# cyrillefavreau/Sol-R

Hardware: AMD Instinct MI355X
Metric: Mrays/s @1920x1080, 3-bounce Cornell (higher is better)
Workload: dtype f32; 1 GPU; cornell 1920x1080, 3 bounces + shadow rays, 75 boxes / 29 primitives, one GPU, whole frame; rays_per_frame=6518779, closest_hit_walks_rank0=3506171, lane_nodes=206382796, lane_prim_tests=37557299, wave_nodes=3396811, wave_prim_tests=626627, wave_walks=106204, cost_ordered_launch_rank0=True, frames_in_flight=3, setup_frames_before_warmup=48, frames_delivered=9105, order_free_nodes=46, short_ray_lists=1, gather=none (one GPU), strips=equal rows, parallelism=tile1

## Files before the change

### sol-r_amd/csrc/build_bounds.h

```cpp
#ifndef SOLR_BUILD_BOUNDS_H
#define SOLR_BUILD_BOUNDS_H

#include <hip/hip_vector_types.h>

#include <cmath>
#include <cstring>

#include "../../include/solr_types.h"

#if defined(__HIPCC__)
#define SOLR_BUILD_BOUNDS_FN __host__ __device__ inline
#else
#define SOLR_BUILD_BOUNDS_FN inline
#endif

namespace solreng
{
#define SOLR_DOMINANT_SHARE 0.25

struct BuildBounds
{
    const float4 *prims = nullptr;
    float margin = 0.f;
    double dominantShare = SOLR_DOMINANT_SHARE;
};

enum BuildBoundsPlainKind
{
    BB_KIND_SHIFT = 24,
    BB_KIND_PLANE_XY = 2,
    BB_KIND_PLANE_YZ = 3,
    BB_KIND_PLANE_XZ = 4
};

SOLR_BUILD_BOUNDS_FN int centreBin(float c, float origin, float scale, int bins)
{
    const float at = (c - origin) * scale;
    const float last = (float)(bins - 1);
    return (int)(at > 0.f ? (at < last ? at : last) : 0.f);
}

SOLR_BUILD_BOUNDS_FN bool leafBuildBounds(const float4 &row0, const float4 &row1, const float4 *prims, int start, int count, float margin,
                                          float lo[3], float hi[3], bool byKind = false)
{
    lo[0] = row0.x, lo[1] = row0.y, lo[2] = row0.z;
    hi[0] = row1.x, hi[1] = row1.y, hi[2] = row0.w;
    if (prims == nullptr || count <= 0 || start < 0)
        return false;
    float lx = INFINITY, ly = INFINITY, lz = INFINITY, hx = -INFINITY, hy = -INFINITY, hz = -INFINITY;
    for (int k = 0; k < count; ++k)
    {
        const float4 p = prims[8 * (size_t)(start + k)], s = prims[8 * (size_t)(start + k) + 1];
        int word;
        memcpy(&word, &p.w, 4);
        const int type = word & 0xff, kind = (word >> BB_KIND_SHIFT) & 15;
        const int across = byKind ? (kind == BB_KIND_PLANE_YZ ? 0 : kind == BB_KIND_PLANE_XZ ? 1 : kind == BB_KIND_PLANE_XY ? 2 : -1)
                                  : (type == ptYZPlane ? 0 : type == ptXZPlane ? 1 : type == ptXYPlane ? 2 : -1);
        if (across < 0)
            return false;
        const float ex = across == 0 ? margin : fabsf(s.x) + margin;
        const float ey = across == 1 ? margin : fabsf(s.y) + margin;
        const float ez = across == 2 ? margin : fabsf(s.z) + margin;
        lx = fminf(lx, p.x - ex), hx = fmaxf(hx, p.x + ex);
        ly = fminf(ly, p.y - ey), hy = fmaxf(hy, p.y + ey);
        lz = fminf(lz, p.z - ez), hz = fmaxf(hz, p.z + ez);
    }
    if (!(lx <= hx && ly <= hy && lz <= hz && fabsf(lx) < 3.0e38f && fabsf(hx) < 3.0e38f && fabsf(ly) < 3.0e38f && fabsf(hy) < 3.0e38f &&
          fabsf(lz) < 3.0e38f && fabsf(hz) < 3.0e38f))
        return false;
    const float nlx = fmaxf(lo[0], lx), nly = fmaxf(lo[1], ly), nlz = fmaxf(lo[2], lz);
    const float nhx = fminf(hi[0], hx), nhy = fminf(hi[1], hy), nhz = fminf(hi[2], hz);
    if (!(nlx <= nhx && nly <= nhy && nlz <= nhz))
        return false;
    lo[0] = nlx, lo[1] = nly, lo[2] = nlz;
    hi[0] = nhx, hi[1] = nhy, hi[2] = nhz;
    return true;
}
}

#endif
```

### sol-r_amd/csrc/engine.h

```cpp
#ifndef SOLR_ENGINE_H
#define SOLR_ENGINE_H

#include <hip/hip_runtime.h>

#include <atomic>
#include <chrono>
#include <cstdio>
#include <cstdlib>
#include <cstring>
#include <string>
#include <vector>

#include "../../include/solr_hip.h"
#include "renderer.h"
#include "lists_device.h"
#include "list_builders.h"

namespace solreng
{
struct HostProfile
{
    const bool on = getenv("SOLR_HIP_HOST_PROFILE") != nullptr;
    struct Entry
    {
// ... 114 lines not shown
    static int ticketOf(long serial, int slot) { return (int)((serial % TICKET_PERIOD) * IMAGE_RING + slot); }
    long imageSerial = 0;
    long slotSerial[IMAGE_RING] = {};
    long shareSeq = 0;
    long slotShareSeq[IMAGE_RING] = {};
    long lastWaitedSeq = 0;
    long sharePublished[IMAGE_RING] = {};
    struct SharedRing *sharedRing = nullptr;
    size_t sharedBytes = 0;
    std::string sharedName;
    int shareRank = 0, shareWorld = 0;
    bool slotOfStrips[IMAGE_RING] = {};
    long lastHandedOut = 0;
    bool copyOnRenderStream = false;
    void release();
};
extern ImageRing gImageRing;
struct CopyLane
{
    hipStream_t stream = nullptr;
    hipEvent_t frameRendered = nullptr;
    hipEvent_t imageDone[ImageRing::IMAGE_RING] = {};
    void release();
};
struct ImageStreaming
{
    int next = 0;
    bool ids = false;
    bool valid = false;
    const void *bitmap = nullptr;
    unsigned serial = 0;
    long key[3] = {0, 0, 0};
    DeviceBuffer counters;
    StreamPlan plan = {};
    int bands = 0;
    unsigned *hostWords = nullptr;
    hipEvent_t rendered = nullptr;
    long delivered = 0;
    int support = -1;
    void release();
};
const int SORT_PERIOD = 64;

struct TileSchedule
{
    int mode = 1;
    DeviceBuffer cost, costSnapshot;
    DeviceBuffer order[2];
    int orderBuffer = 0;
    hipEvent_t orderEvent = nullptr;
    bool orderWait[MAX_FLIGHTS] = {};
    unsigned *hostStats = nullptr;
    unsigned *hostStatsDev = nullptr;
    long key[6] = {0, 0, 0, 0, 0, 0};
    int frames = 0;
    bool reorder = false;
    bool orderValid = false;
    BandCuts orderCuts = {};
    void reset()
    {
        frames = 0;
        reorder = false;
        orderValid = false;
    }
    void release();
};

enum Variant
{
    VARIANT_AUTOMATIC = 0,
    VARIANT_EXACT_LIST = 3,
    VARIANT_ALL_FEATURES = 4,
    VARIANT_NO_GROUPING = 5,
    VARIANT_NO_ORDER_FREE = 6,
    VARIANT_STACK_IN_LDS = 7,
    VARIANT_REFERENCE_LEAVES = 8,
    VARIANT_AO_FIXED_STRIDE = 9,
    VARIANT_NAN_DEEP_STACK = 10,
    VARIANT_UNSORTED_LISTS = 12,
    VARIANT_NO_BAND_WORDS = 13,
    VARIANT_ZERO_STREAM_COUNTERS = 14,
    VARIANT_NO_LAMP_CUTOFF = 15,
    VARIANT_ALL_TRIPS = 16,
    VARIANT_UPLOADED_BUILD_BOXES = 17
};

struct NodeList
{
    int copies, lists;
    explicit NodeList(int copies_ = 1, int lists_ = 1) : copies(copies_), lists(lists_) {}
    std::vector<float4> rows;
    std::vector<int> start, origin;
    int nb = 0;
    unsigned offRows = 0, offLeaf = 0;
    unsigned offStart = 0;
    int ordered = 0;
    bool tight = false;
    std::vector<int> refitLevels;

    void reset() { *this = NodeList(copies, lists); }
    unsigned nodes() const { return (unsigned)lists * (unsigned)nb; }
    unsigned rowsOf(int list) const { return solrdev::listRows(offRows, (unsigned)nb, (unsigned)list); }
    unsigned offThin() const { return solrdev::listThin(offRows, nodes()); }
    unsigned offSorted() const { return solrdev::listSorted(offRows, nodes()); }
    unsigned layRows(unsigned row)
    {
        offRows = row;
        return row + (unsigned)copies * solrdev::listCopyRows(nodes());
    }
    unsigned layStart(unsigned row)
    {
        offStart = row * 4;
        return row + (nodes() + 3u) / 4u;
    }
    unsigned layLeaf(unsigned row)
    {
        row = (row + 3u) & ~3u;
        offLeaf = row;
        return row + 4u * nodes() + 4u;
    }
};


struct Arena
{
    DeviceBuffer geometry;
    unsigned offPrims = 0, offLights = 0;
    unsigned rowsFixed = 0;
    bool geometryDirty = true;
    bool deviceAhead = false;
    void layOutAgain() { geometryDirty = true; }
};
struct OrderFreeState
{
    int freeCountdown = 0;
    bool freeHostValid = true;
    bool freeDirty = false;
    SolrDeviceLists freeStage;
    bool freeStale = false;
    bool sortedFree = false;
    void dropStage(bool originToo)
    {
        if (freeStage.rows)
            (void)hipFree(freeStage.rows);
        if (freeStage.start)
            (void)hipFree(freeStage.start);
        freeStage.rows = nullptr;
        freeStage.start = nullptr;
        if (originToo && freeStage.origin)
        {
            (void)hipFree(freeStage.origin);
            freeStage.origin = nullptr;
        }
    }
};
struct Rotation
{
    DeviceBuffer movable, refitPlan;
    DeviceBuffer enclosesFlag;
    int nbMovable = -1;
    bool refitReady = false;
    bool refitPlanPending = false;
    bool exactStale = false;
    float exactStaleViewDistance = 0.f;
    int nbDeviceRotations = 0;
    int nbDeviceTranslations = 0;
    int nbDeviceLampMoves = 0;
// ... 163 lines not shown
        if (slot < SOLR_MORPH_TRACK_MAX_KEYS)
            ++morph.nbTrackKeys;
    }
    void morphLampNoted(int slotA, int slotB, bool moves)
    {
        if (morph.lampChecked != retags)
            morph.lampAnswers.clear();
        morph.lampChecked = retags;
        morph.lampAnswers.push_back({slotA, slotB, moves});
    }
    void morphServed(bool walkHolds, bool landed, bool track)
    {
        walkEncloses = walkHolds;
        if (landed)
        {
            arena.deviceAhead = true;
            ++(track ? morph.nbDeviceTrackMorphs : morph.nbDeviceMorphs);
        }
    }
    void release()
    {
        lists.dropStage(true);
        for (DeviceBuffer *b : {&arena.geometry, &lamps, &rotation.movable, &rotation.refitPlan, &rotation.enclosesFlag, &rotation.edits,
                                &morph.lampFlag})
            solreng::release(*b);
        for (MorphKey &key : morph.keys)
            solreng::release(key.planes);
        *this = Scene();
    }
};
struct Lights
{
    std::vector<float4> hostLights;
    int nbLights = 0;
};
struct TextureUse
{
    int material;
    long texels;
    long offsets[7];
};
struct Materials
{
    DeviceBuffer table;
    unsigned offMatCold = 0;
    int nbMaterials = 0;
    std::vector<int> materialTags;
    std::vector<float> materialAverage;
    std::vector<TextureUse> textureUses;
    void release()
    {
        solreng::release(table);
        *this = Materials();
    }
};
struct Textures
{
    DeviceBuffer atlas;
    size_t atlasBytes = 0;
    bool textureTablesChecked = false;
    void release()
    {
        solreng::release(atlas);
        *this = Textures();
    }
};
struct Randoms
{
    DeviceBuffer values;
    long nbRandoms = 0;
    float randomsReach = 0.f;
    void release()
    {
        solreng::release(values);
        *this = Randoms();
    }
};
struct SceneFacts
{
    bool primsContained = false;
    bool opaqueShadows = false;
    bool plainPlanes = false;
    float sceneExtent = 1.f;
    int sceneFeatures = F_ALL & ~F_FULL;
};
struct KernelTimer
{
    unsigned timingTick = 0;
    std::vector<std::pair<hipEvent_t, hipEvent_t>> events;
    double timedMs = 0.0;
    int timedLaunches = 0;
    std::vector<float> kernelSamples, intervalSamples;
};
struct WalkRecording
{
    DeviceBuffer walkRecords, walkVisits;
    bool recordNext = false;
    bool recorded = false;
    unsigned recordGrid = 0;
    size_t recordLds = 0;
    int recordVariant = -1;
    bool recordDeep = false;
    SceneArgs recordScene = {};
    void release()
    {
        solreng::release(walkRecords);
        solreng::release(walkVisits);
        *this = WalkRecording();
    }
};

struct Engine
{
    bool initialized = false;
    int device = 0;
    int errorCode = 0;
    std::string errorText;

    int variant = VARIANT_AUTOMATIC;
    bool grouping = true;
    int shortRayListsMode = -1;
    int flights = 1;
    bool tileClocks = false;
    int timing = 0;

    Scene scene;
    Lights lights;
    Materials materials;
    Textures textures;
    Randoms randoms;
    SceneFacts facts;

    DeviceBuffer counters, tileClock;
    DeviceBuffer haloGivenAbove, haloGivenBelow;
    int haloSuppliedAbove = 0, haloSuppliedBelow = 0;
    int haloWanted = -1;
    Flight flight[MAX_FLIGHTS];
    bool ownStream = false;
    bool callerStreams = false;
    int current = 0;
    unsigned frameSerial = 0;
    TileSchedule sched;
    unsigned lastSerial = 0;
    int nbTilesTimed = 0;
    void *boundBitmap = nullptr;
    int width = 0, height = 0;
    int firstRow = 0, nbRows = -1;
    int allocW = 0, allocRows = 0;

    KernelTimer timer;
    WalkRecording recording;

    CopyLane copyLane;
    ImageStreaming streaming;
    int tileCheckedX = 0, tileCheckedTiles = 0, tileCheckedShift = 0;
    unsigned tileCheckedMagic = 0;
    int lastMask = -1;
    int lastFrame[6] = {-1, -1, 0, 0, 0, 0};
};

extern Engine gFirst;
extern Engine *gEngines[SOLR_MAX_GPU_COUNT];
extern int gDevices;
extern int gRequested;
extern Engine *gCurrent;
#define g (*gCurrent)
// ... 45 lines not shown
    fprintf(stderr, "solr_hip: error %d: %s\n", code, buf);
    const char *fatal = getenv("SOLR_HIP_FATAL");
    if (fatal && fatal[0] == '1')
        exit(EXIT_FAILURE);
}

#define HIPCHECK(expr)                                                                                           \
    do                                                                                                           \
    {                                                                                                            \
        hipError_t e_ = (expr);                                                                                  \
        if (e_ != hipSuccess)                                                                                    \
        {                                                                                                        \
            std::string m_ = std::string(#expr) + ": " + hipGetErrorString(e_);                                  \
            setError((int)e_, m_.c_str(), __FILE__, __LINE__);                                                   \
        }                                                                                                        \
    } while (0)

#define ARGCHECK(cond, msg)                                                                                      \
    do                                                                                                           \
    {                                                                                                            \
        if (!(cond))                                                                                             \
            setError(-1, msg, __FILE__, __LINE__);                                                               \
    } while (0)

inline bool ok()
{
    return g.errorCode == 0;
}

inline bool ready(const char *who)
{
    if (!ok())
        return false;
    if (!g.initialized)
    {
        setError(-1, (std::string(who) + ": initialize_scene has not been called").c_str(), __FILE__, __LINE__);
        return false;
    }
    return true;
}

inline void reserve(DeviceBuffer &b, size_t bytes)
{
    if (bytes < 16)
        bytes = 16;
    if (b.ptr && b.bytes >= bytes)
        return;
    release(b);
    HIPCHECK(hipMalloc(&b.ptr, bytes));
    if (ok())
        b.bytes = bytes;
}

template <class T>
void upload(DeviceBuffer &b, const std::vector<T> &host)
{
    reserve(b, host.size() * sizeof(T));
    if (ok() && !host.empty())
    {
        HIPCHECK(hipMemcpyAsync(b.ptr, host.data(), host.size() * sizeof(T), hipMemcpyHostToDevice, sceneStream()));
        HIPCHECK(hipStreamSynchronize(sceneStream()));
    }
}

inline int stripRows()
{
    return g.nbRows >= 0 ? g.nbRows : g.height;
}


void h2dSceneOne(BoundingBox *boundingBoxes, int nbActiveBoxes, Primitive *primitives, int nbPrimitives, Lamp *lamps, int nbLamps);
void h2dMaterialsOne(Material *materials, int nbActiveMaterials);
void h2dRandomsOne(float *randoms);
void h2dRandomsSizedOne(const float *randoms, long count);
void h2dTexturesOne(int activeTextures, TextureInfo *textureInfos);
void h2dLightInformationOne(LightInformation *lightInformation, int lightInformationSize);
void setMovableOne(const unsigned char *flags, int nbPrimitives);
void checkTextureTables();
void maybeBuildOrderFreeLists();
void flushGeometry();
void pullGeometry();
void ensureHostFreeLists();
void buildLeafRecords();
bool listEnclosesInArena(const NodeList &list);
ListKnobs listKnobs();
PruneDecider pruneDecider();
bool orderFreeListsUsable();
bool lampCutoffUsable();
bool shortRayListsChoice();
SceneArgs prepareScene(const SceneInfo &sceneInfo, bool exactNodes);
bool deepNodeList(const SceneArgs &S);
bool canRotateOne(const float center[3], const float cosAngles[3], const float sinAngles[3], float viewDistance,
                  const char *who = "solr_hip_rotate_primitives");
int rotatePrimitivesOne(const float center[3], const float cosAngles[3], const float sinAngles[3], float viewDistance);
bool refitMovedScene(float viewDistance);
void refreshExactList();
int setMorphKeysOne(const Primitive *first, const Primitive *last, int nbPrimitives);
int setMorphTrackKeyOne(int slot, const Primitive *key, const int *rankOf, int nbPrimitives);
bool canMorphOne(int slotA, int slotB, float weight, float viewDistance, const char *who);
int morphKeysOne(int slotA, int slotB, float weight, float viewDistance, const char *who);
bool canTranslateOne(const float translation[3], float viewDistance);
int translatePrimitivesOne(const float translation[3], float viewDistance);
bool canMoveLampOne(int lamp, const float center[3]);
int moveLampOne(int lamp, const float center[3]);
bool canSetPrimitivesOne(const SolrPrimitiveEdit *edits, const int *slots, int n, float viewDistance);
int setPrimitivesOne(const SolrPrimitiveEdit *edits, const int *slots, int n, float viewDistance);
void allocateFrame();
int neededFeatures(const SceneInfo &sceneInfo, bool full);
void renderImpl(const SceneInfo &sceneInfo, const vec4i &objects, const PostProcessingInfo &ppInfo, const float origin[3],
                const float direction[3], const float angles[4], bool counting, unsigned long long counts[8]);
void collectEvents();
void d2hBitmapOne(const SceneInfo &sceneInfo, BitmapBuffer *bitmap, PrimitiveXYIdBuffer *primitivesXYIds, bool wait);
void d2hBitmapWait();
void releaseCopies();
bool imageStreamingCuts(int tileRows, int firstRow[SOLR_STREAM_BANDS_MAX + 1], int *bands, bool withIds);
bool armImageStreaming(FrameArgs &F, int tileRows, hipStream_t stream, bool withIds);
void markStreamedFrame(hipStream_t stream);
void ensureCopyStream();
bool ensureImageRing();
int nextTicket(int *slot);
bool haveCommunicator();
bool communicatorUp();
int agreedHaloRows(const PostProcessingInfo &ppInfo);
void exchangeDepthHalo(int flight, hipStream_t stream, const PixelRecord *pp, int W, int firstRow, int nbRows, int frameRows,
                       int wanted, DepthHalo *halo);
bool shareRandoms();

struct HaloDebt
{
    bool owed = false;
    int wanted = 0, width = 0, frameRows = 0;
    ~HaloDebt()
    {
        if (owed)
            exchangeDepthHalo(g.current, g.flight[g.current].stream, nullptr, width, 0, 0, frameRows, wanted, nullptr);
    }
};
void launchPostProcess(const SceneInfo &sceneInfo, const PostProcessingInfo &ppInfo, int flight, hipStream_t stream, int firstRow,
                       int nbRows, unsigned char *bitmap, HaloDebt &debt);
}

namespace solrmorph
{
void packMorphKeys(hipStream_t stream, const Primitive *key, const int *rankOf, int nbPrimitives, float4 *planes);
}

namespace solrpost
{
void defaultConversion(hipStream_t stream, const SceneInfo &si, int nbPixels, const PixelRecord *pp, unsigned char *bitmap);
void ambientOcclusion(hipStream_t stream, const SceneInfo &si, const PostProcessingInfo &ppi, int nbRows, const PixelRecord *pp,
                      const float *randoms, long nbRandoms, unsigned char *bitmap, const DepthHalo &halo, int firstRow,
                      float randomsReach, bool heavyFirst);
void depthOfField(hipStream_t stream, const SceneInfo &si, const PostProcessingInfo &ppi, int nbRows, const PixelRecord *pp,
                  const float *randoms, long nbRandoms, unsigned char *bitmap);
void radiosity(hipStream_t stream, const SceneInfo &si, const PostProcessingInfo &ppi, int nbRows, const PixelRecord *pp,
               const int4 *ids, const float *randoms, long nbRandoms, unsigned char *bitmap);
void filter(hipStream_t stream, const SceneInfo &si, const PostProcessingInfo &ppi, int nbRows, const PixelRecord *pp,
            unsigned char *bitmap);
void cartoon(hipStream_t stream, const SceneInfo &si, const PostProcessingInfo &ppi, int nbRows, const PixelRecord *pp,
             unsigned char *bitmap);
void orderTiles(hipStream_t stream, const unsigned *cost, unsigned *snapshot, unsigned *order, int nbTiles,
                volatile unsigned *hostStats, int flights, const BandCuts &cuts);
void packDepthRows(hipStream_t stream, const PixelRecord *pp, int W, int row0, int n, float *out);
}

#endif
// ... 1 lines not shown
```

### sol-r_amd/csrc/solr_arena.hip

```cpp
#include <hip/hip_runtime.h>

#include <cmath>

#include "../../include/solr_hip.h"
#include "rt_device.h"

using namespace solrdev;

#include "renderer.h"
#include "engine.h"

using namespace solreng;

namespace solreng
{
__global__ __launch_bounds__(256) void k_buildLeafRecords(float4 *__restrict__ arena, unsigned offNodes, unsigned offStart,
                                                         unsigned offPrims, unsigned offLeaf, int nbNodes)
{
    const int i = blockIdx.x * blockDim.x + threadIdx.x;
    if (i >= nbNodes)
        return;
    float4 r0 = make_float4(0.f, 0.f, 0.f, 0.f), r1 = r0, r2 = r0, r3 = r0;
    const int nb = __float_as_int(arena[offNodes + 2u * (unsigned)i + 1u].z);
    if (nb > 0)
    {
        const int start = ((const int *)arena)[offStart + (unsigned)i];
        const float4 *prim = arena + offPrims + 8u * (unsigned)start;
        r0 = prim[ROW_P0_TYPE];
        r1 = prim[ROW_SIZE_MAT];
        r2 = prim[ROW_P1_INDEX];
        r3 = prim[ROW_P2];
        if (planeClass(__float_as_int(r0.w) & PRIM_TYPE_MASK))
        {
            const float4 n0 = prim[ROW_N0];
            r2 = make_float4(n0.x, n0.y, n0.z, r2.w);
            r3 = make_float4(r3.w, 0.f, 0.f, 0.f);
        }
        r3.w = __int_as_float(start);
    }
    float4 *out = arena + offLeaf + 4u * (unsigned)i;
    out[0] = r0;
    out[1] = r1;
    out[2] = r2;
    out[3] = r3;
}

__global__ __launch_bounds__(256) void k_tightenLeaves(float4 *__restrict__ arena, unsigned offNodes, unsigned offTight,
                                                      unsigned offStart, unsigned offPrims, int nbNodes, float margin)
{
    const int i = blockIdx.x * blockDim.x + threadIdx.x;
    if (i >= nbNodes)
        return;
    float4 row0 = arena[offNodes + 2u * (unsigned)i], row1 = arena[offNodes + 2u * (unsigned)i + 1u];
    const int nb = __float_as_int(row1.z);
    if (nb > 0)
    {
        static_assert(BB_KIND_SHIFT == PRIM_KIND_SHIFT && BB_KIND_PLANE_XY == KIND_PLANE_XY && BB_KIND_PLANE_YZ == KIND_PLANE_YZ &&
                          BB_KIND_PLANE_XZ == KIND_PLANE_XZ && ROW_P0_TYPE == 0 && ROW_SIZE_MAT == 1,
                      "build_bounds.h reads the primitive records as scene_layout.h lays them out");
        const int start = ((const int *)arena)[offStart + (unsigned)i];
        float lo[3], hi[3];
        if (leafBuildBounds(row0, row1, arena + offPrims, start, nb, margin, lo, hi, true))
        {
            row0 = make_float4(lo[0], lo[1], lo[2], hi[2]);
            row1 = make_float4(hi[0], hi[1], row1.z, row1.w);
        }
    }
    arena[offTight + 2u * (unsigned)i] = row0;
    arena[offTight + 2u * (unsigned)i + 1u] = row1;
}

__global__ __launch_bounds__(256) void k_tightenInner(float4 *__restrict__ arena, unsigned offTight, int nbNodes, int listLength)
{
    const int i = blockIdx.x * blockDim.x + threadIdx.x;
    if (i >= nbNodes)
        return;
    const float4 row0 = arena[offTight + 2u * (unsigned)i], row1 = arena[offTight + 2u * (unsigned)i + 1u];
    const int nb = __float_as_int(row1.z), skip = __float_as_int(row1.w);
    if (nb > 0 || skip <= 1)
        return;
    const int listEnd = (i / listLength + 1) * listLength;
    const int end = min(i + skip, listEnd);
    float lx = INFINITY, ly = INFINITY, lz = INFINITY, hx = -INFINITY, hy = -INFINITY, hz = -INFINITY;
    for (int j = i + 1; j < end; ++j)
    {
        const float4 b = arena[offTight + 2u * (unsigned)j + 1u];
        if (__float_as_int(b.z) <= 0)
            continue;
        const float4 a = arena[offTight + 2u * (unsigned)j];
        lx = fminf(lx, a.x), ly = fminf(ly, a.y), lz = fminf(lz, a.z);
        hx = fmaxf(hx, b.x), hy = fmaxf(hy, b.y), hz = fmaxf(hz, a.w);
    }
    const float nlx = fmaxf(row0.x, lx), nly = fmaxf(row0.y, ly), nlz = fmaxf(row0.z, lz);
    const float nhx = fminf(row1.x, hx), nhy = fminf(row1.y, hy), nhz = fminf(row0.w, hz);
    if (!(nlx <= nhx && nly <= nhy && nlz <= nhz))
        return;
    arena[offTight + 2u * (unsigned)i] = make_float4(nlx, nly, nlz, nhz);
    arena[offTight + 2u * (unsigned)i + 1u] = make_float4(nhx, nhy, row1.z, row1.w);
}

__global__ __launch_bounds__(256) void k_listEncloses(const float4 *__restrict__ arena, unsigned offNodes, unsigned offStart,
                                                      unsigned offPrims, int nbNodes, int nbPrims, int *bad)
{
    const int i = blockIdx.x * blockDim.x + threadIdx.x;
    if (i >= nbNodes)
        return;
    const float4 a = arena[offNodes + 2u * (unsigned)i], b = arena[offNodes + 2u * (unsigned)i + 1u];
    const int count = __float_as_int(b.z);
    const int end = min(i + max(__float_as_int(b.w), 1), nbNodes);
    bool encloses = true;
    if (count <= 0)
    {
        for (int j = i + 1; j < end && encloses;)
        {
            const float4 ca = arena[offNodes + 2u * (unsigned)j], cb = arena[offNodes + 2u * (unsigned)j + 1u];
            encloses = ca.x >= a.x && ca.y >= a.y && ca.z >= a.z && cb.x <= b.x && cb.y <= b.y && ca.w <= a.w;
            j += max(__float_as_int(cb.w), 1);
        }
    }
    else
    {
        const int start = ((const int *)arena)[offStart + (unsigned)i];
        for (int k = 0; k < count && encloses; ++k)
        {
            const long long pi = (long long)start + k;
            if (start < 0 || pi >= nbPrims)
            {
                encloses = false;
                break;
            }
            const float4 *r = arena + offPrims + (size_t)PRIM_ROWS * (size_t)pi;
            const float4 p0 = r[ROW_P0_TYPE], size = r[ROW_SIZE_MAT];
            const int type = __float_as_int(p0.w) & PRIM_TYPE_MASK;
            float lo[3] = {p0.x, p0.y, p0.z}, hi[3] = {p0.x, p0.y, p0.z};
            auto add = [&](const float4 &v) {
                lo[0] = v.x < lo[0] ? v.x : lo[0], lo[1] = v.y < lo[1] ? v.y : lo[1], lo[2] = v.z < lo[2] ? v.z : lo[2];
                hi[0] = hi[0] < v.x ? v.x : hi[0], hi[1] = hi[1] < v.y ? v.y : hi[1], hi[2] = hi[2] < v.z ? v.z : hi[2];
            };
            float grow[3] = {size.x, size.y, size.z};
            if (type == ptTriangle)
            {
                add(r[ROW_P1_INDEX]);
                add(r[ROW_P2]);
                grow[0] = grow[1] = grow[2] = 0.f;
            }
            else if (type == ptCylinder)
            {
                add(r[ROW_P1_INDEX]);
                grow[1] = grow[2] = grow[0];
            }
            else if (type == ptSphere)
                grow[1] = grow[2] = grow[0];
            auto larger = [](float x, float y) { return x < y ? y : x; };
            auto slack = [&](int k) { return 4.f * 1.1920929e-7f * larger(larger(fabsf(lo[k]), fabsf(hi[k])), fabsf(grow[k])); };
            const float ex = slack(0), ey = slack(1), ez = slack(2);
            encloses = a.x <= lo[0] - fabsf(grow[0]) + ex && a.y <= lo[1] - fabsf(grow[1]) + ey && a.z <= lo[2] - fabsf(grow[2]) + ez &&
                       b.x >= hi[0] + fabsf(grow[0]) - ex && b.y >= hi[1] + fabsf(grow[1]) - ey && a.w >= hi[2] + fabsf(grow[2]) - ez;
        }
    }
    if (!encloses)
        *bad = 1;
}

void ensureHostFreeLists()
{
    if (g.scene.lists.freeHostValid || !ok())
        return;
    quiesce();
    NodeList &list = g.scene.orderFree;
    const size_t n = list.nodes();
    list.rows.resize(2 * n);
    list.start.resize(n);
    list.origin.resize(n);
    const bool staged = g.scene.lists.freeStage.rows != nullptr;
    const char *arena = (const char *)g.scene.arena.geometry.ptr;
    if (!staged && !arena)
    {
        setError(-1, "order-free lists neither staged nor in the arena", __FILE__, __LINE__);
        return;
    }
    HIPCHECK(hipMemcpy(list.rows.data(), staged ? (const void *)g.scene.lists.freeStage.rows : arena + (size_t)list.offRows * 16, 2 * n * 16,
                       hipMemcpyDeviceToHost));
    HIPCHECK(hipMemcpy(list.start.data(), staged ? (const void *)g.scene.lists.freeStage.start : arena + (size_t)list.offStart * 4, n * 4,
                       hipMemcpyDeviceToHost));
    if (g.scene.lists.freeStage.origin)
        HIPCHECK(hipMemcpy(list.origin.data(), g.scene.lists.freeStage.origin, n * 4, hipMemcpyDeviceToHost));
    if (ok())
    {
        g.scene.hostListsPulled();
    }
}

void pullGeometry()
{
    if (!g.scene.arena.deviceAhead || !g.scene.arena.geometry.ptr)
        return;
    refreshExactList();
    quiesce();
    auto get = [&](unsigned at, void *dst, size_t bytes) {
        if (bytes)
            HIPCHECK(hipMemcpy(dst, (const char *)g.scene.arena.geometry.ptr + (size_t)at * 16, bytes, hipMemcpyDeviceToHost));
    };
    for (NodeList *list : {&g.scene.exact, &g.scene.walk, &g.scene.orderFree})
        if (list != &g.scene.orderFree || g.scene.lists.freeHostValid)
            get(list->offRows, list->rows.data(), list->rows.size() * 16);
    get(g.scene.arena.offPrims, g.scene.hostPrims.data(), g.scene.hostPrims.size() * 16);
    g.scene.hostImagesPulled();
}

static bool tightenList(const NodeList &list)
{
    static const bool off = getenv("SOLR_HIP_NO_TIGHT_LEAVES") != nullptr;
    const int nbNodes = (int)list.nodes(), listLength = list.nb;
    if (off || !g.facts.plainPlanes || nbNodes <= 0 || listLength <= 0 || listLength > 65536 || !ok())
        return false;
    float4 *arena = (float4 *)g.scene.arena.geometry.ptr;
    const float margin = g.facts.sceneExtent * (1.f / 1024.f);
    const dim3 grid((unsigned)((nbNodes + 255) / 256));
    hipLaunchKernelGGL(k_tightenLeaves, grid, dim3(256), 0, sceneStream(), arena, list.offRows, list.offThin(), list.offStart, g.scene.arena.offPrims,
                       nbNodes, margin);
    hipLaunchKernelGGL(k_tightenInner, grid, dim3(256), 0, sceneStream(), arena, list.offThin(), nbNodes, listLength);
    HIPCHECK(hipGetLastError());
    return ok();
}

__global__ __launch_bounds__(256) void k_sortNodeBounds(float4 *__restrict__ arena, unsigned offBoxesFree, unsigned offSorted, int nb)
{
    const int i = blockIdx.x * blockDim.x + threadIdx.x;
    if (i > 8 * nb)
        return;
    float4 a = make_float4(0.f, 0.f, 0.f, 0.f), b = a;
    if (i < 8 * nb)
    {
        const int octant = i / nb;
        a = arena[offBoxesFree + 2u * (unsigned)i];
        b = arena[offBoxesFree + 2u * (unsigned)i + 1u];
        if (octant & 1)
        {
            const float t = a.x;
            a.x = b.x;
            b.x = t;
        }
        if (octant & 2)
        {
            const float t = a.y;
            a.y = b.y;
            b.y = t;
        }
        if (octant & 4)
        {
            const float t = a.z;
            a.z = a.w;
            a.w = t;
        }
        b.w = __int_as_float(__float_as_int(b.w) << 5);
    }
    arena[offSorted + 2u * (unsigned)i] = a;
    arena[offSorted + 2u * (unsigned)i + 1u] = b;
}

static bool sortFreeLists()
{
    static const bool off = getenv("SOLR_HIP_NO_SORTED_LISTS") != nullptr;
    const NodeList &list = g.scene.orderFree;
    if (off || list.nb <= 0 || !ok())
        return false;
    hipLaunchKernelGGL(k_sortNodeBounds, dim3((unsigned)((8 * list.nb + 1 + 255) / 256)), dim3(256), 0, sceneStream(),
                       (float4 *)g.scene.arena.geometry.ptr, list.offRows, list.offSorted(), list.nb);
    HIPCHECK(hipGetLastError());
    return ok();
}

static void deriveList(NodeList &list)
{
    const bool orderFree = &list == &g.scene.orderFree;
    const int n = (orderFree && g.scene.lists.freeStale) ? 0 : (int)list.nodes();
    if (n > 0)
        hipLaunchKernelGGL(k_buildLeafRecords, dim3((unsigned)((n + 255) / 256)), dim3(256), 0, sceneStream(), (float4 *)g.scene.arena.geometry.ptr,
                           list.offRows, list.offStart, g.scene.arena.offPrims, list.offLeaf, n);
    HIPCHECK(hipGetLastError());
    list.tight = list.copies > 1 && n > 0 && tightenList(list);
    if (orderFree)
        g.scene.lists.sortedFree = n > 0 && sortFreeLists();
}

void buildLeafRecords()
{
    if (!ok() || !g.scene.arena.geometry.ptr)
        return;
    for (NodeList *list : {&g.scene.exact, &g.scene.walk, &g.scene.orderFree})
        deriveList(*list);
    HIPCHECK(hipStreamSynchronize(sceneStream()));
}

static void copyStagedLists()
{
    const NodeList &list = g.scene.orderFree;
    char *arena = (char *)g.scene.arena.geometry.ptr;
    const SolrDeviceLists &stage = g.scene.lists.freeStage;
    HIPCHECK(hipMemcpyAsync(arena + (size_t)list.offRows * 16, stage.rows, (size_t)list.nodes() * 32, hipMemcpyDeviceToDevice, sceneStream()));
    HIPCHECK(hipMemcpyAsync(arena + (size_t)list.offStart * 4, stage.start, (size_t)list.nodes() * 4, hipMemcpyDeviceToDevice, sceneStream()));
}

static void appendFreeLists()
{
    const unsigned end = g.scene.orderFree.layLeaf(g.scene.orderFree.layStart(g.scene.orderFree.layRows(g.scene.arena.rowsFixed)));
    const size_t bytes = (size_t)end * 16, fixedBytes = (size_t)g.scene.arena.rowsFixed * 16;
    PhaseTimer phase;
    if (g.scene.arena.geometry.bytes < bytes)
    {
        DeviceBuffer larger;
        reserve(larger, bytes);
        if (!ok())
            return;
        HIPCHECK(hipMemcpyAsync(larger.ptr, g.scene.arena.geometry.ptr, fixedBytes, hipMemcpyDeviceToDevice, sceneStream()));
        HIPCHECK(hipStreamSynchronize(sceneStream()));
        release(g.scene.arena.geometry);
        g.scene.arena.geometry = larger;
    }
    HIPCHECK(hipMemsetAsync((char *)g.scene.arena.geometry.ptr + fixedBytes, 0, bytes - fixedBytes, sceneStream()));
    copyStagedLists();
    if (ok())
        deriveList(g.scene.orderFree);
    HIPCHECK(hipStreamSynchronize(sceneStream()));
    phase.mark("geometry: lists appended");
    if (ok())
        g.scene.listsAppended();
}

void flushGeometry()
{
    if (!g.scene.arena.geometryDirty)
    {
        if (g.scene.lists.freeDirty && g.scene.lists.freeStage.rows && g.scene.arena.geometry.ptr && g.scene.arena.rowsFixed > 0)
            appendFreeLists();
        else if (g.scene.lists.freeDirty)
            g.scene.arena.layOutAgain();
        if (!g.scene.arena.geometryDirty)
            return;
    }
    pullGeometry();
    if (!g.scene.lists.freeStage.rows)
        ensureHostFreeLists();
    unsigned row = g.scene.walk.layRows(g.scene.exact.layRows(0));
    row = (row + 3u) & ~3u;
    g.scene.arena.offPrims = row;
    row += (unsigned)g.scene.hostPrims.size();
    g.scene.arena.offLights = row;
    row += (unsigned)g.lights.hostLights.size();
    row = g.scene.walk.layStart(g.scene.exact.layStart(row));
    row = g.scene.walk.layLeaf(g.scene.exact.layLeaf(row));
    g.scene.arena.rowsFixed = row;
    row = g.scene.orderFree.layLeaf(g.scene.orderFree.layStart(g.scene.orderFree.layRows(row)));
    PhaseTimer phase;
    reserve(g.scene.arena.geometry, (size_t)std::max(row, 1u) * 16);
    if (!ok())
        return;
    HIPCHECK(hipMemsetAsync(g.scene.arena.geometry.ptr, 0, (size_t)std::max(row, 1u) * 16, sceneStream()));
    auto put = [&](unsigned at, const void *src, size_t bytes) {
        if (bytes && ok())
            HIPCHECK(hipMemcpyAsync((char *)g.scene.arena.geometry.ptr + (size_t)at * 16, src, bytes, hipMemcpyHostToDevice, sceneStream()));
    };
    for (const NodeList *list : {&g.scene.exact, &g.scene.walk, &g.scene.orderFree})
        if (list == &g.scene.orderFree && g.scene.lists.freeStage.rows)
        {
            if (ok())
                copyStagedLists();
        }
        else
        {
            put(list->offRows, list->rows.data(), list->rows.size() * 16);
            put(list->offStart / 4, list->start.data(), list->start.size() * 4);
        }
    put(g.scene.arena.offPrims, g.scene.hostPrims.data(), g.scene.hostPrims.size() * 16);
// ... 138 lines not shown
}

bool orderFreeListsUsable()
{
    return g.scene.orderFree.nb > 0 && g.facts.primsContained && !g.scene.lists.freeStale && g.scene.nested && g.scene.walk.ordered &&
           g.variant != VARIANT_NO_ORDER_FREE;
}

bool lampCutoffUsable()
{
    return g.scene.walkEncloses && g.facts.primsContained && g.scene.nested && g.scene.walk.ordered && g.variant != VARIANT_NO_LAMP_CUTOFF;
}

static int tightListsFor(const SceneArgs &S, const SceneInfo &sceneInfo, bool exactNodes)
{
    if (exactNodes || g.variant == VARIANT_REFERENCE_LEAVES || !g.scene.walk.tight || !g.scene.walkEncloses || !sceneInfo.extendedGeometry)
        return 0;
    if (S.nbBoxesFree > 0 && !g.scene.orderFree.tight)
        return 0;
    return (sceneInfo.viewDistance > 0.f && sceneInfo.viewDistance <= 64.f * g.facts.sceneExtent) ? 1 : 0;
}

static bool sortedListsUsable(int nbBoxesFree)
{
    return nbBoxesFree > 0 && g.scene.lists.sortedFree && g.variant != VARIANT_UNSORTED_LISTS;
}

bool shortRayListsChoice()
{
    static const int fromEnv = getenv("SOLR_HIP_SHORT_RAY_LISTS") ? atoi(getenv("SOLR_HIP_SHORT_RAY_LISTS")) : -1;
    const int mode = g.shortRayListsMode >= 0 ? g.shortRayListsMode : fromEnv;
    return mode < 0 ? activeFlights() >= 2 : mode != 0;
}

static SceneArgs makeScene(bool exactNodes)
{
    const NodeList &list = exactNodes ? g.scene.exact : g.scene.walk;
    SceneArgs S;
    memset(&S, 0, sizeof(S));
    S.geometry = g.scene.arena.geometry.ptr;
    S.materials = g.materials.table.ptr;
    S.textures = g.textures.atlas.ptr;
    S.randoms = g.randoms.values.ptr;
    S.offBoxes = list.offRows;
    S.offBoxStart = list.offStart;
    S.offLeaf = list.offLeaf;
    S.offPrims = g.scene.arena.offPrims;
    S.offLights = g.scene.arena.offLights;
    S.offMatCold = g.materials.offMatCold;
    S.nbBoxes = list.nb;
    S.nbPrimitives = g.scene.nbPrimitives;
    S.nbLights = g.lights.nbLights;
    S.nbLamps = g.scene.nbLamps;
    S.nested = g.scene.nested;
    S.orderedBoxes = list.ordered;
    S.nbRandoms = g.randoms.values.ptr ? g.randoms.nbRandoms : 0;
    if (!exactNodes && orderFreeListsUsable())
    {
        S.offBoxesFree = g.scene.orderFree.offRows;
        S.offLeafFree = g.scene.orderFree.offLeaf;
        S.nbBoxesFree = g.scene.orderFree.nb;
        S.opaqueShadows = g.facts.opaqueShadows ? SHADOWS_OPAQUE : 0;
        S.shortRayLists = shortRayListsChoice() ? 1 : 0;
    }
    if (!exactNodes && lampCutoffUsable())
        S.opaqueShadows |= SHADOWS_LAMP_CUTOFF;
    if (g.variant == VARIANT_ALL_TRIPS)
        S.opaqueShadows |= SHADOWS_ALL_TRIPS;
    S.tightLists = 0;
    S.sortedLists = sortedListsUsable(S.nbBoxesFree) ? 1 : 0;
    return S;
}

SceneArgs prepareScene(const SceneInfo &sceneInfo, bool exactNodes)
{
    maybeBuildOrderFreeLists();
    flushGeometry();
    if (exactNodes)
        refreshExactList();
    if (!ok())
        return SceneArgs();
    SceneArgs S = makeScene(exactNodes);
    S.tightLists = tightListsFor(S, sceneInfo, exactNodes);
    return S;
}

bool deepNodeList(const SceneArgs &S)
{
    return S.nbBoxes > 1024;
}

}
```

### sol-r_amd/csrc/solr_moves.hip

```cpp
#include <hip/hip_runtime.h>

#include <cmath>

#include "../../include/solr_hip.h"
#include "rt_device.h"

using namespace solrdev;

#include "renderer.h"
#include "engine.h"

using namespace solreng;

namespace solreng
{
__device__ inline void translateRow(float4 &v, float tx, float ty, float tz)
{
    v.x = v.x + tx;
    v.y = v.y + ty;
    v.z = v.z + tz;
}

__global__ __launch_bounds__(256) void k_translatePrimitives(float4 *__restrict__ arena, unsigned offPrims, int nbPrimitives,
                                                             const unsigned char *__restrict__ movable, float tx, float ty,
// ... 63 lines not shown
    {
        float4 *p0 = arena + M.offPrims + (size_t)PRIM_ROWS * M.lamp + ROW_P0_TYPE;
        float4 *location = arena + M.offLights + 3u * (unsigned)M.lamp;
        p0->x = M.x, p0->y = M.y, p0->z = M.z;
        location->x = M.x, location->y = M.y, location->z = M.z;
    }
    for (int l = 0; l < 3; ++l)
    {
        const LeafRecordsOf &L = M.list[l];
        if (t < L.nodes)
        {
            const int nb = __float_as_int(arena[L.offRows + 2u * (unsigned)t + 1u].z);
            if (nb > 0 && ((const int *)arena)[L.offStart + (unsigned)t] == M.lamp)
            {
                float4 *record = arena + L.offLeaf + 4u * (unsigned)t;
                record->x = M.x, record->y = M.y, record->z = M.z;
            }
            return;
        }
        t -= L.nodes;
    }
}

bool canMoveLampOne(int lamp, const float center[3])
{
    if (!g.initialized || !ok())
        return false;
    const Scene &s = g.scene;
    const char *why = nullptr;
    if (s.nbPrimitives <= 0 || s.hostPrims.size() < (size_t)PRIM_ROWS * (size_t)s.nbPrimitives || s.exact.nb <= 0 || s.exact.start.empty() ||
        s.exact.rows.size() < 2)
        why = "no resident scene";
    else if (lamp < 0 || lamp >= s.nbLamps || lamp >= s.nbPrimitives)
        why = "no such lamp";
    else if (!center || !std::isfinite(center[0]) || !std::isfinite(center[1]) || !std::isfinite(center[2]))
        why = "no centre, or a component that is not finite";
    else if (g.lights.nbLights < s.nbLamps || g.lights.hostLights.size() < 3 * (size_t)s.nbLamps ||
             bitsi(g.lights.hostLights[3 * (size_t)lamp].w) != bitsi(s.hostPrims[(size_t)PRIM_ROWS * lamp + ROW_P1_INDEX].w))
        why = "the light records are not the lamps'";
    else
    {
        const float4 a = s.exact.rows[0], b = s.exact.rows[1];
        const float grow = fabsf(s.hostPrims[(size_t)PRIM_ROWS * lamp + ROW_SIZE_MAT].x);
        const int type = bitsi(s.hostPrims[(size_t)PRIM_ROWS * lamp + ROW_P0_TYPE].w) & PRIM_TYPE_MASK;
        if (s.exact.start[0] > lamp || (long)s.exact.start[0] + bitsi(b.z) <= lamp || type != ptSphere)
            why = "not a sphere of the first cell";
        else if (!(a.x <= center[0] - grow && a.y <= center[1] - grow && a.z <= center[2] - grow && b.x >= center[0] + grow &&
                   b.y >= center[1] + grow && a.w >= center[2] + grow))
            why = "the lamp would leave its cell";
    }
    if (why && getenv("SOLR_HIP_DEBUG_TREE"))
        fprintf(stderr, "solr_hip_move_lamp refused: %s (lamp %d of %d, %d light records)\n", why, lamp, s.nbLamps, g.lights.nbLights);
    return why == nullptr;
}

int moveLampOne(int lamp, const float center[3])
{
    if (!canMoveLampOne(lamp, center))
        return 0;
    HIPCHECK(hipSetDevice(g.device));
    flushGeometry();
    if (!ok() || !g.scene.arena.geometry.ptr)
        return 0;
    quiesce();
    LampMove M;
    int total = 1;
    int l = 0;
    for (const NodeList *list : {&g.scene.exact, &g.scene.walk, &g.scene.orderFree})
    {
        const bool none = list == &g.scene.orderFree && g.scene.lists.freeStale;
        M.list[l].offRows = list->offRows;
        M.list[l].offStart = list->offStart;
        M.list[l].offLeaf = list->offLeaf;
        M.list[l].nodes = none ? 0 : (int)list->nodes();
        total += M.list[l].nodes;
        ++l;
    }
    M.offPrims = g.scene.arena.offPrims;
    M.offLights = g.scene.arena.offLights;
    M.lamp = lamp;
    M.x = center[0], M.y = center[1], M.z = center[2];
    hipLaunchKernelGGL(k_moveLamp, dim3((unsigned)((total + 255) / 256)), dim3(256), 0, sceneStream(), (float4 *)g.scene.arena.geometry.ptr, M);
    HIPCHECK(hipGetLastError());
    HIPCHECK(hipStreamSynchronize(sceneStream()));
    if (ok())
    {
        float4 &p0 = g.scene.hostPrims[(size_t)PRIM_ROWS * lamp + ROW_P0_TYPE], &location = g.lights.hostLights[3 * (size_t)lamp];
        p0.x = location.x = center[0];
        p0.y = location.y = center[1];
        p0.z = location.z = center[2];
    }
    g.scene.lampMoveServed(ok());
    return ok() ? 1 : 0;
}

}

extern "C" {
int solr_hip_device_translations(void)
{
    return g.scene.rotation.nbDeviceTranslations;
}

int solr_hip_device_lamp_moves(void)
{
    return g.scene.rotation.nbDeviceLampMoves;
}

int solr_hip_read_lights(float *rows, int capacityRows)
{
    if (!ready("solr_hip_read_lights") || !g.scene.arena.geometry.ptr)
        return -1;
    flushGeometry();
    quiesce();
    const int n = (int)g.lights.hostLights.size();
    if (!rows)
        return n;
    if (n > capacityRows)
        return -1;
    if (n)
        HIPCHECK(hipMemcpy(rows, (const char *)g.scene.arena.geometry.ptr + (size_t)g.scene.arena.offLights * 16, (size_t)n * 16,
                           hipMemcpyDeviceToHost));
    return ok() ? n : -1;
}
}
```

### sol-r_amd/csrc/solr_uploads.hip

```cpp
#include <hip/hip_runtime.h>

#include <cmath>

#include "../../include/solr_hip.h"
#include "rt_device.h"

using namespace solrdev;

#include "renderer.h"
#include "engine.h"

using namespace solreng;

namespace solreng
{
static_assert((int)LB_ROW_P0_TYPE == (int)ROW_P0_TYPE && (int)LB_ROW_SIZE_MAT == (int)ROW_SIZE_MAT &&
                  (int)LB_ROW_P1_INDEX == (int)ROW_P1_INDEX && (int)LB_ROW_P2 == (int)ROW_P2 && (int)LB_PRIM_ROWS == (int)PRIM_ROWS &&
                  (int)LB_PRIM_TYPE_MASK == (int)PRIM_TYPE_MASK,
              "list_builders.h and scene_layout.h disagree about the primitive record");

int materialTag(const Material &m)
{
    int tag = 0;
    if (m.attributes.x == 0)
        tag |= PRIM_FAST0;
    if (m.attributes.x == 1)
        tag |= PRIM_FAST1;
    if (m.attributes.y != 0)
        tag |= PRIM_PROCEDURAL;
    if (m.transparency != 0.f)
        tag |= PRIM_TRANSPARENT;
    if (m.attributes.z == 1)
        tag |= PRIM_WIRE1;
    if (m.attributes.z == 2)
        tag |= PRIM_WIRE2;
    if (m.innerIllumination.x != 0.f)
        tag |= PRIM_EMISSIVE;
    if (m.textureIds.x != TEXTURE_NONE)
        tag |= PRIM_TEXTURED;
    int w = m.attributes.w;
    w = w < -1 ? -1 : (w > 100 ? 100 : w);
    tag |= (w + 1) << PRIM_WIDTH_SHIFT;
    return tag;
}

void retagPrimitives()
{
    pullGeometry();
    const size_t n = g.scene.hostPrims.size() / PRIM_ROWS;
    const bool noKinds = getenv("SOLR_HIP_NO_KINDS") != nullptr;
    int features = 0;
    bool contained = true, opaque = true, planes = false;
    float extent = 1.f;
    for (size_t i = 0; i < n; ++i)
    {
        float4 *r = &g.scene.hostPrims[PRIM_ROWS * i];
        for (int row : {(int)ROW_P0_TYPE, (int)ROW_P1_INDEX, (int)ROW_P2})
            for (float c : {r[row].x, r[row].y, r[row].z})
                if (fabsf(c) < 3.0e38f)
                    extent = std::max(extent, fabsf(c));
        int tag, mat;
        memcpy(&tag, &r[ROW_P0_TYPE].w, 4);
        memcpy(&mat, &r[ROW_SIZE_MAT].w, 4);
        const int type = tag & PRIM_TYPE_MASK;
        const int facts = (mat >= 0 && (size_t)mat < g.materials.materialTags.size()) ? g.materials.materialTags[mat]
                                                                                      : (PRIM_FAST0 | (1 << PRIM_WIDTH_SHIFT));
        int kind = KIND_GENERAL;
        if (noKinds || !(facts & PRIM_FAST0))
            kind = KIND_GENERAL;
        else if (type == ptSphere && !(facts & PRIM_PROCEDURAL))
            kind = KIND_SPHERE;
        else if ((type == ptXYPlane || type == ptYZPlane || type == ptXZPlane) && !(facts & (PRIM_TEXTURED | PRIM_WIRE2)) &&
                 !(type == ptYZPlane && (facts & PRIM_EMISSIVE)))
            kind = type == ptXYPlane ? KIND_PLANE_XY : (type == ptYZPlane ? KIND_PLANE_YZ : KIND_PLANE_XZ);
        else if (type == ptTriangle)
            kind = KIND_TRIANGLE;
        else if (type == ptCylinder || type == ptCone)
            kind = KIND_CYLINDER;
        r[ROW_P0_TYPE].w = bitsf(type | facts | (kind << PRIM_KIND_SHIFT));
        planes = planes || kind == KIND_PLANE_XY || kind == KIND_PLANE_YZ || kind == KIND_PLANE_XZ;
        opaque = opaque && !(facts & PRIM_TRANSPARENT) && !(facts & PRIM_TEXTURED) && type != ptCamera;
        contained = contained && (type == ptTriangle || type == ptCylinder || (type == ptSphere && !(facts & PRIM_PROCEDURAL)) ||
                                  type == ptXYPlane || type == ptYZPlane || type == ptXZPlane);
        r[ROW_P2].w = (mat >= 0 && (size_t)mat < g.materials.materialAverage.size()) ? g.materials.materialAverage[mat] : 0.f;
        switch (type)
        {
        case ptSphere:
        case ptEnvironment:
            features |= (facts & PRIM_PROCEDURAL) ? F_PROC : F_SPHERE;
            break;
        case ptCylinder:
        case ptCone:
            features |= F_CYL;
            break;
        case ptEllipsoid:
            features |= F_ELL;
            break;
        case ptTriangle:
            features |= F_TRI;
            break;
        case ptCamera:
            features |= F_PLANE | F_TEX;
            break;
        default:
            features |= F_PLANE;
            break;
        }
        if (facts & PRIM_TEXTURED)
            features |= F_TEX;
    }
    float reach = 0.f;
    for (size_t i = 0; i < n; ++i)
        for (float c : {g.scene.hostPrims[PRIM_ROWS * i + ROW_SIZE_MAT].x, g.scene.hostPrims[PRIM_ROWS * i + ROW_SIZE_MAT].y,
                        g.scene.hostPrims[PRIM_ROWS * i + ROW_SIZE_MAT].z})
            if (fabsf(c) < 3.0e38f)
                reach = std::max(reach, fabsf(c));
    g.facts.sceneExtent = extent + reach;
    g.facts.plainPlanes = planes;
    g.facts.sceneFeatures = features;
    g.facts.primsContained = contained && n > 0;
    g.facts.opaqueShadows = opaque && n > 0;
    g.scene.retagged();
    g.scene.arena.layOutAgain();
}

void checkTextureTables()
{
    if (g.textures.textureTablesChecked)
        return;
    g.textures.textureTablesChecked = true;
    for (const TextureUse &use : g.materials.textureUses)
    {
        ARGCHECK(use.texels > 0, "cudaRender: a textured material with an empty or negative texture mapping");
        ARGCHECK(g.textures.atlas.ptr != nullptr && g.textures.atlasBytes > 0,
                 "cudaRender: textured materials but no texture atlas was uploaded (h2d_textures)");
        for (int t = 0; ok() && t < 7; ++t)
            if (use.offsets[t] >= 0 || t == 0)
                ARGCHECK(use.offsets[t] >= 0 && (size_t)(use.offsets[t] + use.texels + 2) <= g.textures.atlasBytes,
                         "cudaRender: a material's texture table points outside the uploaded atlas");
        if (!ok())
        {
            g.textures.textureTablesChecked = false;
            return;
        }
    }
}


void h2dSceneOne(BoundingBox *boundingBoxes, int nbActiveBoxes, Primitive *primitives, int nbPrimitives, Lamp *lamps,
                        int nbLamps)
{
    if (!ready("h2d_scene"))
        return;
    quiesce();
    ARGCHECK(nbActiveBoxes >= 0 && nbPrimitives >= 0 && nbLamps >= 0, "h2d_scene: negative count");
    ARGCHECK(nbActiveBoxes == 0 || boundingBoxes, "h2d_scene: null boxes");
    ARGCHECK(nbPrimitives == 0 || primitives, "h2d_scene: null primitives");
    if (!ok())
        return;
    PhaseTimer phase;
    std::vector<float4> boxes(2 * (size_t)nbActiveBoxes);
    std::vector<int> start(nbActiveBoxes);
    for (int i = 0; i < nbActiveBoxes; ++i)
    {
        const BoundingBox &b = boundingBoxes[i];
        ARGCHECK(b.nbPrimitives >= 0 && (b.nbPrimitives == 0 || (b.startIndex >= 0 &&
                                                                  (long)b.startIndex + b.nbPrimitives <= nbPrimitives)),
                 "h2d_scene: box primitive range outside the primitive array");
        boxes[2 * i] = make_float4(b.parameters[0].x, b.parameters[0].y, b.parameters[0].z, b.parameters[1].z);
        boxes[2 * i + 1] =
            make_float4(b.parameters[1].x, b.parameters[1].y, bitsf(b.nbPrimitives), bitsf(b.indexForNextBox.x));
        start[i] = b.startIndex;
    }
    if (!ok())
        return;
    phase.mark("h2d_scene: node rows");
    const int nested = validateNesting(boundingBoxes, nbActiveBoxes);
    phase.mark("h2d_scene: nesting check");
    if (!nested)
    {
        for (int i = 0; i < nbActiveBoxes; ++i)
            ARGCHECK(boundingBoxes[i].indexForNextBox.x >= 1, "h2d_scene: skip pointer < 1");
        if (!ok())
            return;
    }

    std::vector<float4> boxesC;
    std::vector<int> startC, originC;
    const int nc = collapseChains(boxes, start, nested != 0, boxesC, startC, originC, &g.scene.exact.ordered, &g.scene.walk.ordered);

    int freeCountdown = 0;
    if (nested && g.scene.walk.ordered && nc > 1 && g.grouping && !getenv("SOLR_HIP_NO_FREE_ORDER"))
        freeCountdown = std::max(1, getenv("SOLR_HIP_FREE_AFTER") ? atoi(getenv("SOLR_HIP_FREE_AFTER")) : 2);

    int nbWalkNodes = nc, prunedBefore = 0, prunedAfter = 0;
    if (nested && g.scene.walk.ordered && nc > 0 && g.grouping)
    {
        phase.mark("h2d_scene: chain collapse");
        nbWalkNodes = buildWalkOrderList(boxesC, startC, originC, listKnobs(), pruneDecider(), &prunedBefore, &prunedAfter,
                                         [&](const char *what) { phase.mark((std::string("h2d_scene: ") + what).c_str()); });
    }
// ... 311 lines not shown
```

Baseline: 30760 Mrays/s.

## Tighten leaf bounds around sphere-only leaves with precision-safe padding

Extends the leaf-tightening pass so leaves holding only spheres get boxes shrunk to the spheres' extents. The padding is conservative and scales with view distance and scene reach. The goal is fewer node visits and primitive tests when uploaded leaf boxes are looser than the spheres they hold. A host-side check detects loose sphere leaves, and the lists are re-tightened when the view distance changes or a lamp moves, which adds a quiesce and re-launch at those points.

```diff
diff --git a/sol-r_amd/csrc/build_bounds.h b/sol-r_amd/csrc/build_bounds.h
--- a/sol-r_amd/csrc/build_bounds.h
+++ b/sol-r_amd/csrc/build_bounds.h
@@ -28,6 +28,7 @@
 enum BuildBoundsPlainKind
 {
     BB_KIND_SHIFT = 24,
+    BB_KIND_SPHERE = 1,
     BB_KIND_PLANE_XY = 2,
     BB_KIND_PLANE_YZ = 3,
     BB_KIND_PLANE_XZ = 4
@@ -40,14 +41,22 @@
     return (int)(at > 0.f ? (at < last ? at : last) : 0.f);
 }
 
+SOLR_BUILD_BOUNDS_FN float sphereBuildExtent(const float4 &p, float radius, float margin, float reach)
+{
+    const float r = fabsf(radius);
+    const float far = reach + fmaxf(fmaxf(fabsf(p.x), fabsf(p.y)), fabsf(p.z));
+    return ((r + margin) + (3.f * far * 0x1p-21f) / (r / far)) + far * 0x1p-9f;
+}
+
 SOLR_BUILD_BOUNDS_FN bool leafBuildBounds(const float4 &row0, const float4 &row1, const float4 *prims, int start, int count, float margin,
-                                          float lo[3], float hi[3], bool byKind = false)
+                                          float lo[3], float hi[3], bool byKind = false, float reach = 0.f)
 {
     lo[0] = row0.x, lo[1] = row0.y, lo[2] = row0.z;
     hi[0] = row1.x, hi[1] = row1.y, hi[2] = row0.w;
     if (prims == nullptr || count <= 0 || start < 0)
         return false;
     float lx = INFINITY, ly = INFINITY, lz = INFINITY, hx = -INFINITY, hy = -INFINITY, hz = -INFINITY;
+    bool spheres = false;
     for (int k = 0; k < count; ++k)
     {
         const float4 p = prims[8 * (size_t)(start + k)], s = prims[8 * (size_t)(start + k) + 1];
@@ -56,11 +65,19 @@
         const int type = word & 0xff, kind = (word >> BB_KIND_SHIFT) & 15;
         const int across = byKind ? (kind == BB_KIND_PLANE_YZ ? 0 : kind == BB_KIND_PLANE_XZ ? 1 : kind == BB_KIND_PLANE_XY ? 2 : -1)
                                   : (type == ptYZPlane ? 0 : type == ptXZPlane ? 1 : type == ptXYPlane ? 2 : -1);
-        if (across < 0)
+        const bool sphere = reach > 0.f && byKind && kind == BB_KIND_SPHERE;
+        if ((across < 0 && !sphere) || (k > 0 && sphere != spheres))
             return false;
-        const float ex = across == 0 ? margin : fabsf(s.x) + margin;
-        const float ey = across == 1 ? margin : fabsf(s.y) + margin;
-        const float ez = across == 2 ? margin : fabsf(s.z) + margin;
+        spheres = sphere;
+        float ex = across == 0 ? margin : fabsf(s.x) + margin;
+        float ey = across == 1 ? margin : fabsf(s.y) + margin;
+        float ez = across == 2 ? margin : fabsf(s.z) + margin;
+        if (sphere)
+        {
+            ex = ey = ez = sphereBuildExtent(p, s.x, margin, reach);
+            if (!(ex < 3.0e38f && fabsf(p.x) < 3.0e38f && fabsf(p.y) < 3.0e38f && fabsf(p.z) < 3.0e38f))
+                return false;
+        }
         lx = fminf(lx, p.x - ex), hx = fmaxf(hx, p.x + ex);
         ly = fminf(ly, p.y - ey), hy = fmaxf(hy, p.y + ey);
         lz = fminf(lz, p.z - ez), hz = fmaxf(hz, p.z + ez);
diff --git a/sol-r_amd/csrc/engine.h b/sol-r_amd/csrc/engine.h
--- a/sol-r_amd/csrc/engine.h
+++ b/sol-r_amd/csrc/engine.h
@@ -220,7 +220,8 @@
     VARIANT_ZERO_STREAM_COUNTERS = 14,
     VARIANT_NO_LAMP_CUTOFF = 15,
     VARIANT_ALL_TRIPS = 16,
-    VARIANT_UPLOADED_BUILD_BOXES = 17
+    VARIANT_UPLOADED_BUILD_BOXES = 17,
+    VARIANT_UPLOADED_SPHERE_LEAVES = 18
 };
 
 struct NodeList
@@ -550,6 +551,9 @@
     bool opaqueShadows = false;
     bool plainPlanes = false;
     float sceneExtent = 1.f;
+    bool looseSpheres = false;
+    float thinReach = 0.f;
+    float frameViewDistance = 0.f;
     int sceneFeatures = F_ALL & ~F_FULL;
 };
 struct KernelTimer
@@ -761,6 +765,8 @@
 void pullGeometry();
 void ensureHostFreeLists();
 void buildLeafRecords();
+void tightenListsAgain();
+float thinReachWanted(float viewDistance);
 bool listEnclosesInArena(const NodeList &list);
 ListKnobs listKnobs();
 PruneDecider pruneDecider();
diff --git a/sol-r_amd/csrc/solr_arena.hip b/sol-r_amd/csrc/solr_arena.hip
--- a/sol-r_amd/csrc/solr_arena.hip
+++ b/sol-r_amd/csrc/solr_arena.hip
@@ -46,7 +46,7 @@
 }
 
 __global__ __launch_bounds__(256) void k_tightenLeaves(float4 *__restrict__ arena, unsigned offNodes, unsigned offTight,
-                                                      unsigned offStart, unsigned offPrims, int nbNodes, float margin)
+                                                      unsigned offStart, unsigned offPrims, int nbNodes, float margin, float reach)
 {
     const int i = blockIdx.x * blockDim.x + threadIdx.x;
     if (i >= nbNodes)
@@ -56,11 +56,11 @@
     if (nb > 0)
     {
         static_assert(BB_KIND_SHIFT == PRIM_KIND_SHIFT && BB_KIND_PLANE_XY == KIND_PLANE_XY && BB_KIND_PLANE_YZ == KIND_PLANE_YZ &&
-                          BB_KIND_PLANE_XZ == KIND_PLANE_XZ && ROW_P0_TYPE == 0 && ROW_SIZE_MAT == 1,
+                          BB_KIND_PLANE_XZ == KIND_PLANE_XZ && BB_KIND_SPHERE == KIND_SPHERE && ROW_P0_TYPE == 0 && ROW_SIZE_MAT == 1,
                       "build_bounds.h reads the primitive records as scene_layout.h lays them out");
         const int start = ((const int *)arena)[offStart + (unsigned)i];
         float lo[3], hi[3];
-        if (leafBuildBounds(row0, row1, arena + offPrims, start, nb, margin, lo, hi, true))
+        if (leafBuildBounds(row0, row1, arena + offPrims, start, nb, margin, lo, hi, true, reach))
         {
             row0 = make_float4(lo[0], lo[1], lo[2], hi[2]);
             row1 = make_float4(hi[0], hi[1], row1.z, row1.w);
@@ -208,17 +208,25 @@
     g.scene.hostImagesPulled();
 }
 
+float thinReachWanted(float viewDistance)
+{
+    if (g.variant == VARIANT_UPLOADED_SPHERE_LEAVES)
+        return 0.f;
+    return viewDistance > g.facts.sceneExtent ? viewDistance : g.facts.sceneExtent;
+}
+
 static bool tightenList(const NodeList &list)
 {
     static const bool off = getenv("SOLR_HIP_NO_TIGHT_LEAVES") != nullptr;
     const int nbNodes = (int)list.nodes(), listLength = list.nb;
-    if (off || !g.facts.plainPlanes || nbNodes <= 0 || listLength <= 0 || listLength > 65536 || !ok())
+    const bool worth = g.facts.plainPlanes || (g.facts.looseSpheres && (g.facts.sceneFeatures & F_PLANE) != 0);
+    if (off || !worth || nbNodes <= 0 || listLength <= 0 || listLength > 65536 || !ok())
         return false;
     float4 *arena = (float4 *)g.scene.arena.geometry.ptr;
     const float margin = g.facts.sceneExtent * (1.f / 1024.f);
     const dim3 grid((unsigned)((nbNodes + 255) / 256));
     hipLaunchKernelGGL(k_tightenLeaves, grid, dim3(256), 0, sceneStream(), arena, list.offRows, list.offThin(), list.offStart, g.scene.arena.offPrims,
-                       nbNodes, margin);
+                       nbNodes, margin, g.facts.thinReach);
     hipLaunchKernelGGL(k_tightenInner, grid, dim3(256), 0, sceneStream(), arena, list.offThin(), nbNodes, listLength);
     HIPCHECK(hipGetLastError());
     return ok();
@@ -290,6 +298,16 @@
         return;
     for (NodeList *list : {&g.scene.exact, &g.scene.walk, &g.scene.orderFree})
         deriveList(*list);
+    HIPCHECK(hipStreamSynchronize(sceneStream()));
+}
+
+void tightenListsAgain()
+{
+    if (!ok() || !g.scene.arena.geometry.ptr)
+        return;
+    for (NodeList *list : {&g.scene.walk, &g.scene.orderFree})
+        if (list->tight)
+            list->tight = tightenList(*list);
     HIPCHECK(hipStreamSynchronize(sceneStream()));
 }
 
@@ -594,6 +612,15 @@
         return SceneArgs();
     SceneArgs S = makeScene(exactNodes);
     S.tightLists = tightListsFor(S, sceneInfo, exactNodes);
+    g.facts.frameViewDistance = sceneInfo.viewDistance;
+    if (S.tightLists && thinReachWanted(sceneInfo.viewDistance) != g.facts.thinReach)
+    {
+        quiesce();
+        g.facts.thinReach = thinReachWanted(sceneInfo.viewDistance);
+        tightenListsAgain();
+        if (!ok())
+            return SceneArgs();
+    }
     return S;
 }
 
diff --git a/sol-r_amd/csrc/solr_moves.hip b/sol-r_amd/csrc/solr_moves.hip
--- a/sol-r_amd/csrc/solr_moves.hip
+++ b/sol-r_amd/csrc/solr_moves.hip
@@ -169,6 +169,7 @@
     M.x = center[0], M.y = center[1], M.z = center[2];
     hipLaunchKernelGGL(k_moveLamp, dim3((unsigned)((total + 255) / 256)), dim3(256), 0, sceneStream(), (float4 *)g.scene.arena.geometry.ptr, M);
     HIPCHECK(hipGetLastError());
+    tightenListsAgain();
     HIPCHECK(hipStreamSynchronize(sceneStream()));
     if (ok())
     {
diff --git a/sol-r_amd/csrc/solr_uploads.hip b/sol-r_amd/csrc/solr_uploads.hip
--- a/sol-r_amd/csrc/solr_uploads.hip
+++ b/sol-r_amd/csrc/solr_uploads.hip
@@ -50,7 +50,7 @@
     const size_t n = g.scene.hostPrims.size() / PRIM_ROWS;
     const bool noKinds = getenv("SOLR_HIP_NO_KINDS") != nullptr;
     int features = 0;
-    bool contained = true, opaque = true, planes = false;
+    bool contained = true, opaque = true, planes = false, spheres = false;
     float extent = 1.f;
     for (size_t i = 0; i < n; ++i)
     {
@@ -79,6 +79,7 @@
             kind = KIND_CYLINDER;
         r[ROW_P0_TYPE].w = bitsf(type | facts | (kind << PRIM_KIND_SHIFT));
         planes = planes || kind == KIND_PLANE_XY || kind == KIND_PLANE_YZ || kind == KIND_PLANE_XZ;
+        spheres = spheres || kind == KIND_SPHERE;
         opaque = opaque && !(facts & PRIM_TRANSPARENT) && !(facts & PRIM_TEXTURED) && type != ptCamera;
         contained = contained && (type == ptTriangle || type == ptCylinder || (type == ptSphere && !(facts & PRIM_PROCEDURAL)) ||
                                   type == ptXYPlane || type == ptYZPlane || type == ptXZPlane);
@@ -117,6 +118,29 @@
                 reach = std::max(reach, fabsf(c));
     g.facts.sceneExtent = extent + reach;
     g.facts.plainPlanes = planes;
+    bool loose = false;
+    const std::vector<float4> &rows = g.scene.exact.rows;
+    const std::vector<int> &start = g.scene.exact.start;
+    for (size_t i = 0; spheres && !loose && i < start.size() && 2 * i + 1 < rows.size(); ++i)
+    {
+        const float4 a = rows[2 * i], b = rows[2 * i + 1];
+        const int count = bitsi(b.z);
+        if (count <= 0 || start[i] < 0 || (size_t)start[i] + (size_t)count > n)
+            continue;
+        bool all = true;
+        float lo[3] = {INFINITY, INFINITY, INFINITY}, hi[3] = {-INFINITY, -INFINITY, -INFINITY};
+        for (int k = 0; k < count && all; ++k)
+        {
+            const float4 p = g.scene.hostPrims[PRIM_ROWS * ((size_t)start[i] + k) + ROW_P0_TYPE];
+            const float r = fabsf(g.scene.hostPrims[PRIM_ROWS * ((size_t)start[i] + k) + ROW_SIZE_MAT].x);
+            all = ((bitsi(p.w) >> PRIM_KIND_SHIFT) & 15) == KIND_SPHERE;
+            lo[0] = std::min(lo[0], p.x - r), lo[1] = std::min(lo[1], p.y - r), lo[2] = std::min(lo[2], p.z - r);
+            hi[0] = std::max(hi[0], p.x + r), hi[1] = std::max(hi[1], p.y + r), hi[2] = std::max(hi[2], p.z + r);
+        }
+        loose = all && (a.x < lo[0] || a.y < lo[1] || a.z < lo[2] || b.x > hi[0] || b.y > hi[1] || a.w > hi[2]);
+    }
+    g.facts.looseSpheres = loose;
+    g.facts.thinReach = thinReachWanted(g.facts.frameViewDistance);
     g.facts.sceneFeatures = features;
     g.facts.primsContained = contained && n > 0;
     g.facts.opaqueShadows = opaque && n > 0;
```

Measured after the change: 31670 Mrays/s, median of 6. +3.0%, better.
